# ecml-peagnn/graph_recsys_benchmark

Hardware: AMD Instinct MI355X
Metric: BPR-scored edges/sec, PEAGAT MovieLens-25m, emb_dim=64, 9 metapaths (higher is better)
Workload: dtype f32; 1 GPU; ml25m_shaped PEAGAT forward+BPR: N=273744 nodes, 9 metapaths x 2 steps, 208376439 messages/step, emb 64 / hidden 64 / repr 16, batch 4096 triples; headline=True, parallelism=single

## Files before the change

graph_recsys_benchmark_amd/_lib.py:

```python
import ctypes as C
import os

_HERE = os.path.dirname(os.path.abspath(__file__))
LIB_PATH = os.environ.get('PEA_LIB') or os.path.join(_HERE, 'csrc', 'libpeahip.so')

PEA_OK = 0
KIND_GAT, KIND_GCN, KIND_SAGE = 0, 1, 2
PLAN_SELF_LOOPS = 1
PLAN_EDGE_IDS = 2
FUSE_ATT, FUSE_MEAN = 0, 1
KG_KGAT, KG_KGCN = 0, 1

_ERR_NAMES = {-1: 'bad argument', -2: 'id out of range', -3: 'HIP runtime error', -4: 'workspace too small',
              -5: 'no gfx950 device'}


class PeaError(RuntimeError):
    def __init__(self, code, msg):
        super().__init__('peahip error %d (%s): %s' % (code, _ERR_NAMES.get(code, '?'), msg))
        self.code = code


class ModelDesc(C.Structure):
    _fields_ = [('kind', C.c_int), ('num_channels', C.c_int), ('steps', C.POINTER(C.c_int)),
# ... 9 lines not shown
                ('src_col', C.c_int)]


class GwJob(C.Structure):
    _fields_ = [('a', C.c_void_p), ('lda', C.c_int64), ('ma', C.c_int), ('b', C.c_void_p), ('ldb', C.c_int64),
                ('nb', C.c_int), ('out', C.c_void_p), ('ldo', C.c_int64), ('b_mask', C.c_void_p), ('b_alt', C.c_void_p),
                ('ldb_alt', C.c_int64), ('b_alt_scale', C.c_void_p)]


class XchgJob(C.Structure):
    _fields_ = [('table', C.c_void_p), ('ld', C.c_int64), ('col', C.c_int), ('width', C.c_int), ('nodes', C.c_void_p),
                ('slots', C.c_void_p), ('n', C.c_int64), ('buf_off', C.c_int64), ('slots_per_rank', C.c_int)]


class DenseJob(C.Structure):
    _fields_ = [('a', C.c_void_p), ('lda', C.c_int64), ('k', C.c_int), ('w', C.c_void_p), ('ldw', C.c_int64),
                ('n_out', C.c_int), ('out', C.c_void_p), ('ldo', C.c_int64), ('gate', C.c_void_p), ('ld_gate', C.c_int64)]


class DenseRouteEntry(C.Structure):
    _fields_ = [('name', C.c_char * 32), ('family', C.c_int), ('variant', C.c_int), ('listed', C.c_int), ('col_group', C.c_int),
                ('lds_bytes', C.c_int64), ('n_jobs', C.c_int), ('job', C.c_int * 12), ('col0', C.c_int * 12),
                ('n_out', C.c_int * 12), ('gate_col0', C.c_int * 12)]


class Mlp2BwdChan(C.Structure):
    _fields_ = [('w0', C.c_void_p), ('w1', C.c_void_p), ('dt1_col', C.c_int), ('h_col', C.c_int), ('dz_col', C.c_int),
                ('da_col', C.c_int)]


class Mlp2BwdChanSage(C.Structure):
    _fields_ = [('w0_root', C.c_void_p), ('w1_root', C.c_void_p), ('dr1_col', C.c_int), ('dxr_col', C.c_int)]


class StageOpts(C.Structure):
    _fields_ = [('part', C.c_int), ('sel_ids', C.c_void_p), ('sel_stride', C.c_int64), ('n_sel', C.c_int64),
                ('sel_out', C.c_void_p), ('err_flag', C.c_void_p)]


PART_ALL, PART_SOURCES, PART_REST = 0, 1, 2
BWD_PREMASKED = 0x100

_vp, _i64, _int, _sz = C.c_void_p, C.c_int64, C.c_int, C.c_size_t
SIGNATURES = {
    'pea_version': (C.c_char_p, []),
    'pea_last_error': (C.c_char_p, []),
# ... 40 lines not shown
    'pea_edge_softmax_backward': (_int, [_vp, _int, _vp, _vp, _vp, _vp, _sz, _vp]),
    'pea_kg_edge_types': (_int, [_vp, _int, _vp, _i64, _int, _vp, _vp]),
    'pea_kg_attention_workspace_bytes': (_sz, [_vp, _int, _int, _int]),
    'pea_kg_attention': (_int, [_vp, _int, _int, _int, _vp, _i64, _vp, _vp, _vp, _vp, _vp, _sz, _vp]),
    'pea_grad_weight_workspace_bytes': (_sz, []),
    'pea_grad_weight': (_int, [_i64, _int, C.POINTER(GwJob), _vp, _sz, _vp]),
    'pea_dense_batch': (_int, [_i64, _int, C.POINTER(DenseJob), _vp]),
    'pea_mlp2_backward_data_workspace_bytes': (_sz, [_int, _int, _int, _int]),
    'pea_mlp2_backward_data': (_int, [_i64, _int, C.POINTER(Mlp2BwdChan), _int, _int, _int, _vp, _i64, _vp, _i64, _vp, _i64, _vp,
                                      _i64, _vp, _vp, _int, _vp, _sz, _vp]),
    'pea_rows_nonzero_workspace_bytes': (_sz, [_i64]),
    'pea_rows_nonzero': (_int, [_i64, _int, _vp, _i64, _vp, _vp, _vp, _vp, _sz, _vp]),
    'pea_rows_nonzero_or': (_int, [_i64, _int, _vp, _i64, _vp, _vp, _vp, _vp, _vp, _sz, _vp]),
    'pea_mlp2_backward_data_sage': (_int, [_i64, _int, C.POINTER(Mlp2BwdChan), C.POINTER(Mlp2BwdChanSage), _int, _int, _int,
                                           _vp, _i64, _vp, _i64, _vp, _i64, _vp, _i64, _vp, _i64, _vp, _i64, _vp, _vp, _vp, _sz,
                                           _vp]),
    'pea_grad_weight_rows': (_int, [_i64, _vp, _vp, _i64, _int, C.POINTER(GwJob), _vp, _sz, _vp]),
    'pea_model_set_active_rows0': (_int, [_vp, _vp, _vp, _vp]),
    'pea_rows_zero': (_int, [_vp, _i64, _int, _vp, _vp, _vp]),
    'pea_block_sum': (_int, [_i64, _int, _int, _vp, _i64, _vp, _i64, _vp]),
    'pea_grad_weight_sharded': (_int, [_i64, _int, _int, _int, _int, C.POINTER(GwJob), _vp, _sz, _vp]),
    'pea_dense_batch_rows': (_int, [_i64, _vp, _int, C.POINTER(DenseJob), _vp]),
    'pea_dense_route': (_int, [_i64, _int, _int, C.POINTER(DenseJob), _int, C.POINTER(DenseRouteEntry), C.POINTER(_int)]),
    'pea_sample_negatives': (_int, [_i64, _int, _vp, _vp, _i64, _i64, _vp, _i64, C.c_uint64, C.c_uint32, _vp, _i64, _vp, _vp]),
    'pea_fuse': (_int, [_i64, _int, _int, _vp, _i64, C.POINTER(_int), _vp, _int, _int, _vp, _vp]),
    'pea_bpr_workspace_bytes': (_sz, [_i64]),
    'pea_bpr_score': (_int, [_i64, _int, _i64, _vp, _vp, _i64, _vp, _vp, _vp, _vp, _vp, _vp, _vp, _vp, _sz, _vp]),
    'pea_predict': (_int, [_i64, _int, _i64, _vp, _vp, _vp, _vp, _vp, _vp, _vp, _vp, _vp]),
    'pea_profile_enable': (_int, [_int]),
    'pea_profile_read': (_int, [_int, C.c_char_p, C.POINTER(C.c_float), C.POINTER(C.c_double), C.POINTER(_int)]),
    'pea_profile_read_ex': (_int, [_int, C.c_char_p, C.POINTER(C.c_float), C.POINTER(C.c_double), C.POINTER(C.c_double),
                                   C.POINTER(C.c_double), C.POINTER(_int)]),
    'pea_entity_reg_workspace_bytes': (C.c_size_t, [_i64, _int]),
    'pea_entity_reg': (_int, [_i64, _int, _i64, _vp, _i64, _vp, _i64, _vp, _vp, _vp, C.c_size_t, _vp]),
    'pea_bpr_train_workspace_bytes': (C.c_size_t, [_i64]),
    'pea_bpr_train_supported': (_int, [_int, _int]),
    'pea_bpr_train': (_int, [_i64, _int, _int, _vp, _i64, _vp, _vp, _vp, _vp, _vp, _vp, _vp, _vp, _vp, _vp, _vp, C.c_size_t, _vp]),
    'pea_rows_scatter_sum_workspace_bytes': (C.c_size_t, [_i64]),
    'pea_rows_scatter_sum': (_int, [_i64, _vp, _vp, _i64, _int, _int, C.POINTER(_int), _vp, _i64, _i64, _vp, C.c_size_t, _vp]),
    'pea_rows_pack': (_int, [_vp, _i64, _int, _int, _vp, _i64, _vp, _i64, _vp]),
    'pea_rows_unpack': (_int, [_vp, _i64, _vp, _int, _vp, _i64, _vp, _i64, _int, _vp]),
    'pea_rows_pack_batch': (_int, [_int, C.POINTER(XchgJob), _vp, _vp]),
    'pea_rows_unpack_batch': (_int, [_int, C.POINTER(XchgJob), _vp, _i64, _vp]),
    'pea_rows_select_owned': (_int, [_vp, _i64, _int, _i64, _vp, _i64, _i64, _int, _int, _int, _vp, _vp, _vp]),
    'pea_rank_eval': (_int, [_i64, _int, _int, _i64, _vp, _vp, _vp, _vp, _vp, _vp, _vp, _vp, _vp, _vp, _vp, _vp]),
    'pea_fuse_ablate': (_int, [_i64, _int, _int, _vp, _i64, C.POINTER(_int), _vp, _int, _vp, _vp, _vp]),
# ... 28 lines not shown
            fn.argtypes = args
        _lib = lib
    return _lib


def last_error():
    return load().pea_last_error().decode()


def check(rc):
    if rc != PEA_OK:
        raise PeaError(rc, last_error())


def dense_route(n_rows, rows_given, jobs):
    lib = load()
    cnt = C.c_int()
    check(lib.pea_dense_route(n_rows, int(rows_given), len(jobs), jobs, 0, None, C.byref(cnt)))
    out = (DenseRouteEntry * max(cnt.value, 1))()
    check(lib.pea_dense_route(n_rows, int(rows_given), len(jobs), jobs, cnt.value, out, C.byref(cnt)))
    return list(out[:cnt.value])


def require_device():
    lib = load()
    if lib.pea_device_count() <= 0:
        raise PeaError(-5, 'no gfx950 (MI355X) device visible; the HIP path has no CPU fallback')
    return lib


class Tape:

    def __init__(self):
        self._h = C.c_void_p()
        check(load().pea_tape_create(C.byref(self._h)))

    def record(self):
        return _TapeRecording(self)

    def replay(self):
        check(load().pea_tape_replay(self._h, current_stream()))

    def __len__(self):
        return int(load().pea_tape_length(self._h))

    def __del__(self):
# ... 37 lines not shown
```

graph_recsys_benchmark_amd/csrc/agg.hip:

```cpp
#include <algorithm>
#include <cstdlib>

#include "agg_common.h"

namespace pea {

namespace {

template <int MODE>
__device__ __forceinline__ void finish_row(const AggGroup &P, int row, int c4, int deg, Soft st, float4 sum) {
    float4 o;
    if (MODE == AGG_GAT) {
        const float inv = 1.0f / (st.s + 1e-16f);
        o = scale4(st.acc, inv);
        if (P.stats && c4 % P.F == 0) {
            float *sp = P.stats + (size_t)row * P.ld_stats + 2 * (c4 / P.F);
            sp[0] = st.m;
            sp[1] = st.s;
        }
    } else if (MODE == AGG_GCN || MODE == AGG_WSUM) {
        o = sum;
    } else {
        const float inv = 1.0f / (float)(deg < 1 ? 1 : deg);
        o = scale4(sum, inv);
// ... 237 lines not shown
        }
    }
    if (sub == 0 && active) finish_row<MODE>(P, row, c4, it.end - it.beg, st, sum);
}

template <int G, int MODE, int F4T>
__global__ __launch_bounds__(kBlock) void agg_rows_kernel(const AggLaunch L) {
    if ((int)blockIdx.x >= L.n_long_blocks) {
        const int b = (int)blockIdx.x - L.n_long_blocks;
        int gi = 0;
        while (gi + 1 < L.n_groups && b >= L.blk_short[gi + 1]) ++gi;
        short_rows<G, MODE, F4T>(L.g[gi], b - L.blk_short[gi]);
        return;
    }
    const int gi = find_group(L);
    const AggGroup &P = L.g[gi];
    const int wave = (int)threadIdx.x / kWave;
    const int lane = (int)threadIdx.x % kWave;
    const int item = ((int)blockIdx.x - L.blk_start[gi]) * (kBlock / kWave) + wave;
    if (item >= P.n_long) return;
    const LongItem it = P.long_items[item];
    if (it.slot == -2) return;
    long_item<G, MODE, F4T, 4, false>(P, it, lane, nullptr, nullptr);
}

template <int G, int MODE, int HL, int V4>
__device__ __forceinline__ void long_item_fat(const AggGroup &P, const LongItem it, const int lane) {
    constexpr int NSG = kWave / G, U = 4, V = 4 * V4;
    const int sub = lane / G, sl = lane % G;
    const bool active = sl * V < P.W;
    const int pos = sl % HL;
    const int c0 = active ? (sl / HL) * P.F + 4 * pos : 0;
    constexpr int CS = 4 * HL;
    const float *feat = P.feat + c0;
    const float *feat_self = P.feat_self + c0;
    const int row = it.row;
    const int kk = 2 * (c0 / P.F);

    float sm = kNegBig, ss = 0.f;
    float4 acc[V4];
#pragma unroll
    for (int v = 0; v < V4; ++v) acc[v] = make_float4(0.f, 0.f, 0.f, 0.f);
    float a_d = 0.f, di = 0.f;
    const float slope = P.neg_slope;
    float4 att_s[V4], h_self[V4];
    if (MODE == AGG_GAT) {
// ... 252 lines not shown
        } else if (MODE == AGG_GCN) {
            const float di = P.dinv_self[row];
            sum = fma4(di * di, h, sum);
        }
    }
    const int deg = P.rowptr[row + 1] - P.rowptr[row];
    if (sub == 0 && active) finish_row<MODE>(P, row, c4, deg, st, sum);
}


template <int G, int MODE>
const char *kname(int which) {
    static char names[4][32];
    static bool init = false;
    if (!init) {
        const char *w[4] = {"short", "rows", "merge", "longhot"};
        const char *m = MODE == AGG_GAT ? "gat" : MODE == AGG_GCN ? "gcn" : MODE == AGG_WSUM ? "wsum" : "mean";
        for (int i = 0; i < 4; ++i) snprintf(names[i], sizeof(names[i]), "agg_%s_g%d_%s", w[i], G, m);
        init = true;
    }
    return names[which];
}

template <int G, int MODE, int F4T>
int launch_for_g(const AggLaunch &base, const int *sel, int n_sel, hipStream_t stream) {
    AggLaunch L;
    double bytes_short = 0.0;
    double pull_short = 0.0, table = 0.0;
    for (int i = 0; i < n_sel; ++i) {
        const AggGroup &g = base.g[sel[i]];
        const double per_msg = 4.0 * g.W + 4.0 * g.idx_share + (MODE == AGG_GAT ? 4.0 * (g.W / g.F) : MODE == AGG_GCN ? 4.0 * g.idx_share : 0.0);
        bytes_short += per_msg * g.msgs_short;
        const double pull = 4.0 * g.W + 4.0 + (MODE == AGG_GCN ? 4.0 : 0.0);
        pull_short += pull * g.msgs_short;
        table = table > g.table_rows * 4.0 * g.W ? table : g.table_rows * 4.0 * g.W;
    }
    L.n_groups = 0;
    int blocks = 0, sblocks = 0;
    double pull_plain = 0.0, alg_plain = 0.0;
    for (int i = 0; i < n_sel; ++i) {
        const AggGroup &g = base.g[sel[i]];
        const bool long_here = g.n_long > 0 && !g.hot_col && !g.skip_long;
        if (g.n_short <= 0 && !long_here) continue;
        L.blk_start[L.n_groups] = blocks;
        L.blk_short[L.n_groups] = sblocks;
        AggGroup &c = L.g[L.n_groups++];
        c = g;
        if (!long_here) c.n_long = 0;
        if (g.n_short > 0) sblocks += (g.n_short + (kBlock / G) - 1) / (kBlock / G);
        if (!long_here) continue;
        blocks += ((g.n_long + 3) / 4 + 7) / 8 * 8;
        const double per_msg = 4.0 * g.W + 4.0 * g.idx_share + (MODE == AGG_GAT ? 4.0 * (g.W / g.F) : MODE == AGG_GCN ? 4.0 * g.idx_share : 0.0);
        alg_plain += per_msg * g.msgs_long;
        pull_plain += (4.0 * g.W + 4.0 + (MODE == AGG_GCN ? 4.0 : 0.0)) * g.msgs_long;
    }
    L.blk_start[L.n_groups] = blocks;
    L.blk_short[L.n_groups] = sblocks;
    L.n_long_blocks = blocks;
    if (blocks + sblocks > 0) {
        ProfScope ps(kname<G, MODE>(1), stream, alg_plain + bytes_short, pull_plain + pull_short, table);
        PEA_LAUNCH((agg_rows_kernel<G, MODE, F4T>), dim3(blocks + sblocks), dim3(kBlock), 0, stream, L);
        PEA_HIP(hipGetLastError());
    }
    for (int i = 0; i < n_sel; ++i) {
        const AggGroup &g = base.g[sel[i]];
        if (g.n_long <= 0 || !g.hot_col || g.skip_long) continue;
        if (MODE == AGG_WSUM) return PEA_ERR_ARG;
        L.n_groups = 1;
        L.blk_start[0] = 0;
        L.g[0] = g;
        const size_t lds = (size_t)g.hot_K * g.W * sizeof(float) + (MODE == AGG_GCN ? (size_t)g.hot_K * sizeof(float) : 0);
        static size_t lds_set = 0;
        if (lds > lds_set) {
            PEA_HIP(hipFuncSetAttribute(reinterpret_cast<const void *>(&agg_long_hot_kernel<G, MODE, F4T>),
                                        hipFuncAttributeMaxDynamicSharedMemorySize, (int)lds));
            lds_set = lds;
        }
        const int n_virtual = (g.n_long + 3) / 4;
        const int grid = std::max(8, std::min(256, (n_virtual + 3) / 4 + 7 & ~7));
        const double per_msg = 4.0 * g.W + 4.0 * g.idx_share + (MODE == AGG_GAT ? 4.0 * (g.W / g.F) : MODE == AGG_GCN ? 4.0 * g.idx_share : 0.0);
        const double pull = (4.0 * g.W + (MODE == AGG_GCN ? 4.0 : 0.0)) * g.msgs_long * (1.0 - g.hot_frac) + 4.0 * g.msgs_long +
                            (double)grid * (double)lds;
        ProfScope ps(kname<G, MODE>(3), stream, per_msg * g.msgs_long, pull, g.table_rows * 4.0 * g.W);
        PEA_LAUNCH((agg_long_hot_kernel<G, MODE, F4T>), dim3(grid), dim3(kHotBlock), lds, stream, L);
        PEA_HIP(hipGetLastError());
    }
    L.n_groups = 0;
    blocks = 0;
    for (int i = 0; i < n_sel; ++i) {
        const AggGroup &g = base.g[sel[i]];
        if (g.n_hub <= 0) continue;
        L.blk_start[L.n_groups] = blocks;
        L.g[L.n_groups++] = g;
        blocks += (g.n_hub + 3) / 4;
    }
    L.blk_start[L.n_groups] = blocks;
    if (blocks > 0) {
        ProfScope ps(kname<G, MODE>(2), stream, 0.0);
        PEA_LAUNCH((agg_merge_kernel<G, MODE, F4T>), dim3(blocks), dim3(kBlock), 0, stream, L);
        PEA_HIP(hipGetLastError());
    }
    return PEA_OK;
}

int f4_class(int mode, int G, int F) {
    if (mode != AGG_GAT) return 0;
    const int f4 = F / 4;
    return f4 == G ? G : f4 == 4 ? 4 : 0;
}

template <int G, int MODE>
int launch_g(const AggLaunch &base, int cls, const int *sel, int n, hipStream_t stream) {
    if (MODE == AGG_GAT && cls == G) return launch_for_g<G, MODE, G>(base, sel, n, stream);
    if (MODE == AGG_GAT && cls == 4) return launch_for_g<G, MODE, (G >= 4 ? 4 : 0)>(base, sel, n, stream);
    return launch_for_g<G, MODE, 0>(base, sel, n, stream);
}

template <int MODE>
const char *fat_name(int G) {
    static char names[4][32];
    const int i = G == 8 ? 0 : G == 16 ? 1 : G == 32 ? 2 : 3;
    if (!names[i][0]) {
        const char *m = MODE == AGG_GAT ? "gat" : MODE == AGG_GCN ? "gcn" : "mean";
        snprintf(names[i], sizeof(names[i]), "agg_long_fat_g%d_%s", G, m);
    }
    return names[i];
}

template <int G, int MODE, int HL, int V4>
int launch_fat(const AggLaunch &base, const int *sel, int n_sel, hipStream_t stream) {
    AggLaunch L;
    L.n_groups = 0;
    int blocks = 0;
    double alg = 0.0, pull = 0.0, table = 0.0;
    for (int i = 0; i < n_sel; ++i) {
        const AggGroup &g = base.g[sel[i]];
        L.blk_start[L.n_groups] = blocks;
        L.g[L.n_groups++] = g;
// ... 32 lines not shown
    }
    for (int c = 0; c < 6; ++c) {
        int sel[kMaxAggGroups], n = 0;
        for (int i = 0; i < base.n_groups; ++i)
            if (cls[i] == c) sel[n++] = i;
        if (!n) continue;
        switch (c) {
            case 0: PEA_TRY((launch_fat<8, MODE, 8, 2>(base, sel, n, stream))); break;
            case 1: PEA_TRY((launch_fat<16, MODE, 8, 2>(base, sel, n, stream))); break;
            case 2: PEA_TRY((launch_fat<32, MODE, 8, 2>(base, sel, n, stream))); break;
            case 3: PEA_TRY((launch_fat<8, MODE, 8, 4>(base, sel, n, stream))); break;
            case 4: PEA_TRY((launch_fat<16, MODE, 8, 4>(base, sel, n, stream))); break;
            default: PEA_TRY((launch_fat<16, MODE, 16, 4>(base, sel, n, stream))); break;
        }
        for (int q = 0; q < n; ++q) base.g[sel[q]].skip_long = 1;
    }
    return PEA_OK;
}

template <int MODE>
int launch_mode(const AggLaunch &base_in, hipStream_t stream) {
    AggLaunch base = base_in;
    PEA_TRY(launch_fat_groups<MODE>(base, stream));
    const int classes[3] = {0, 4, -1};
    for (int G = 4; G <= 64; G <<= 1) {
        for (int ci = 0; ci < 3; ++ci) {
            const int cls = classes[ci] < 0 ? G : classes[ci];
            if (ci == 1 && G == 4) continue;
            int sel[kMaxAggGroups], n = 0;
            for (int i = 0; i < base.n_groups; ++i)
                if (lanes_for(base.g[i].W) == G && f4_class(MODE, G, base.g[i].F) == cls) sel[n++] = i;
            if (!n) continue;
            switch (G) {
                case 4: PEA_TRY((launch_g<4, MODE>(base, cls, sel, n, stream))); break;
                case 8: PEA_TRY((launch_g<8, MODE>(base, cls, sel, n, stream))); break;
                case 16: PEA_TRY((launch_g<16, MODE>(base, cls, sel, n, stream))); break;
                case 32: PEA_TRY((launch_g<32, MODE>(base, cls, sel, n, stream))); break;
                default: PEA_TRY((launch_g<64, MODE>(base, cls, sel, n, stream))); break;
            }
        }
    }
    return PEA_OK;
}

}

size_t partial_record_floats(int W, int F) { return (size_t)W + 2 * (size_t)(W / F); }

int launch_aggregate(AggMode mode, const AggGroup *groups, int n_groups, hipStream_t stream) {
    PEA_REQUIRE(n_groups >= 0 && n_groups <= kMaxAggGroups, PEA_ERR_ARG, "aggregate: %d groups (max %d)",
                n_groups, kMaxAggGroups);
    AggLaunch base;
    base.n_groups = n_groups;
    for (int i = 0; i < n_groups; ++i) {
        const AggGroup &g = groups[i];
        PEA_REQUIRE(g.W > 0 && g.W <= 256 && g.W % 4 == 0, PEA_ERR_ARG,
                    "aggregate: group width %d must be a multiple of 4 in (0, 256]", g.W);
        PEA_REQUIRE(g.F > 0 && g.F % 4 == 0 && g.W % g.F == 0, PEA_ERR_ARG,
                    "aggregate: head width %d must be a multiple of 4 dividing %d", g.F, g.W);
        PEA_REQUIRE(g.ld_feat % 4 == 0 && g.ld_out % 4 == 0, PEA_ERR_ARG,
                    "aggregate: row strides must be multiples of 4 floats");
        PEA_REQUIRE(g.n_hub == 0 || g.partial != nullptr, PEA_ERR_ARG, "aggregate: hub rows need a partial buffer");
        PEA_REQUIRE(mode != AGG_GAT || (g.neg_slope >= 0.f && g.neg_slope <= 1.f), PEA_ERR_ARG,
                    "aggregate: negative_slope %g outside [0, 1] is not supported", (double)g.neg_slope);
        base.g[i] = g;
    }
    switch (mode) {
        case AGG_GAT: return launch_mode<AGG_GAT>(base, stream);
        case AGG_GCN: return launch_mode<AGG_GCN>(base, stream);
        case AGG_WSUM: return launch_mode<AGG_WSUM>(base, stream);
        default: return launch_mode<AGG_MEAN>(base, stream);
    }
}

}
```

graph_recsys_benchmark_amd/csrc/agg_common.h:

```cpp
#pragma once
#include "common.h"

namespace pea {
namespace {

constexpr int kBlock = 256;
constexpr float kNegBig = -3.0e38f;
constexpr float kLog2e = 1.44269504088896340736f;

struct AggLaunch {
    int n_groups;
    int blk_start[kMaxAggGroups + 1];
    int n_long_blocks;
    int blk_short[kMaxAggGroups + 1];
    AggGroup g[kMaxAggGroups];
};

__device__ __forceinline__ float4 ld4(const float *p) { return *reinterpret_cast<const float4 *>(p); }
__device__ __forceinline__ void st4(float *p, float4 v) { *reinterpret_cast<float4 *>(p) = v; }
__device__ __forceinline__ float4 fma4(float w, float4 h, float4 a) {
    return make_float4(fmaf(w, h.x, a.x), fmaf(w, h.y, a.y), fmaf(w, h.z, a.z), fmaf(w, h.w, a.w));
}
__device__ __forceinline__ float4 scale4(float4 a, float f) { return make_float4(a.x * f, a.y * f, a.z * f, a.w * f); }
__device__ __forceinline__ float4 add4(float4 a, float4 b) { return make_float4(a.x + b.x, a.y + b.y, a.z + b.z, a.w + b.w); }
__device__ __forceinline__ float4 shfl_xor4(float4 v, int m) {
    return make_float4(__shfl_xor(v.x, m), __shfl_xor(v.y, m), __shfl_xor(v.z, m), __shfl_xor(v.w, m));
}

struct Soft {
    float m, s;
    float4 acc;
    __device__ __forceinline__ void init() { m = kNegBig; s = 0.f; acc = make_float4(0.f, 0.f, 0.f, 0.f); }
    __device__ __forceinline__ void push(float e, float4 h) {
        const float mn = fmaxf(m, e * kLog2e);
        const float fs = __builtin_amdgcn_exp2f(m - mn);
        const float p = __builtin_amdgcn_exp2f(fmaf(e, kLog2e, -mn));
        m = mn;
// ... 66 lines not shown
```

graph_recsys_benchmark_amd/csrc/common.h:

```cpp
#pragma once
#include <hip/hip_runtime.h>

#include <cstdarg>
#include <cstdint>
#include <cstdio>
#include <functional>
#include <string>
#include <vector>

#include "../../include/peahip.h"

namespace pea {

void set_error(const char *fmt, ...);
const char *get_error();

#define PEA_HIP(call)                                                                          \
    do {                                                                                       \
        hipError_t e_ = (call);                                                                \
        if (e_ != hipSuccess) {                                                                \
            pea::set_error("%s:%d: %s failed: %s", __FILE__, __LINE__, #call,                 \
                           hipGetErrorString(e_));                                             \
            return PEA_ERR_HIP;                                                                \
        }                                                                                      \
// ... 187 lines not shown
    m.rank = rank;
    if ((tile & (tile - 1)) == 0) {
        m.shift = 0;
        while ((1 << m.shift) < tile) ++m.shift;
    }
    const int64_t tiles = (N + tile - 1) / tile;
    const int64_t own_tiles = tiles > rank ? (tiles - rank + world - 1) / world : 0;
    m.n = own_tiles * tile;
    return m;
}

inline RowMap make_rowmap_list(int64_t N, const int *list, const int *count_dev, int64_t capacity) {
    RowMap m;
    m.N = N;
    m.n = capacity;
    m.list = list;
    m.count = count_dev;
    return m;
}

constexpr int kMaxAggGroups = 16;
int launch_aggregate(AggMode mode, const AggGroup *groups, int n_groups, hipStream_t stream);
size_t partial_record_floats(int W, int F);
constexpr int kColsumParts = 512;
int launch_gat_backward(AggMode mode, const AggGroup *groups, int n_groups, hipStream_t stream);
int launch_colsum(const RowMap &rows, int W, int F, const float *A, int lda, const float *S, int lds, float scale, float *part,
                  float *out, hipStream_t stream);
int launch_colsum2(const RowMap &rows, int W, int F, const float *A, int lda, const float *S0, const float *S1, int lds,
                   float scale, float *part, float *out0, float *out1, hipStream_t stream);
int launch_relu_mask(const RowMap &rows, int W, float *G, int ldg, const float *O, int ldo, hipStream_t stream);

struct GemmSegment {
    int c0, c1;
    float *dst;
    int ld;
    int relu;
    const float *gate;
    int ld_gate;
};
constexpr int kMaxSegments = 4;
struct GemmJob {
    const unsigned char *a1_mask;
    const float *a1_alt, *a1_bias, *a1_scale;
    int lda_alt;
    const float *A1;
    const float *A2;
// ... 120 lines not shown
```

include/peahip.h:

```cpp
#ifndef PEAHIP_H_
#define PEAHIP_H_

#include <stddef.h>
#include <stdint.h>

#ifdef __cplusplus
extern "C" {
#endif

#define PEA_OK 0
#define PEA_ERR_ARG (-1)
#define PEA_ERR_RANGE (-2)
#define PEA_ERR_HIP (-3)
#define PEA_ERR_NOMEM (-4)
#define PEA_ERR_DEVICE (-5)

#define PEA_KIND_GAT 0
#define PEA_KIND_GCN 1
#define PEA_KIND_SAGE 2

#define PEA_PLAN_SELF_LOOPS 1

#define PEA_PLAN_EDGE_IDS 2

// ... 92 lines not shown
int pea_block_sum(int64_t n_rows, int n_blocks, int width, const float *src, int64_t ld, float *dst, int64_t ld_dst,
                  void *stream);
int pea_grad_weight_sharded(int64_t n_rows, int shard_tile, int shard_world, int shard_rank, int n_jobs,
                            const pea_gw_job *jobs_host, void *workspace, size_t workspace_bytes, void *stream);
int pea_dense_batch_rows(int64_t n_rows, const int32_t *rows, int n_jobs, const pea_dense_job *jobs_host, void *stream);
#define PEA_ROUTE_SKINNY 0
#define PEA_ROUTE_PERSIST 1
#define PEA_ROUTE_DEEP_RESIDENT 2
#define PEA_ROUTE_DEEP_CHUNK 3
#define PEA_ROUTE_DEEP_STAGED 4
#define PEA_ROUTE_MAX_JOBS 12
typedef struct pea_dense_route_entry {
    char name[32];
    int family, variant;
    int listed;
    int col_group;
    int64_t lds_bytes;
    int n_jobs;
    int job[PEA_ROUTE_MAX_JOBS], col0[PEA_ROUTE_MAX_JOBS], n_out[PEA_ROUTE_MAX_JOBS], gate_col0[PEA_ROUTE_MAX_JOBS];
} pea_dense_route_entry;
int pea_dense_route(int64_t n_rows, int rows_given, int n_jobs, const pea_dense_job *jobs_host, int cap,
                    pea_dense_route_entry *entries_out, int *count_out);

int pea_sample_negatives(int64_t n_pos, int k, const int64_t *pos_u, const int64_t *pos_i, int64_t item_lo,
                         int64_t num_items, const int64_t *seen_keys_sorted, int64_t n_keys, uint64_t seed,
                         uint32_t offset, int64_t *out_triples, int64_t ld_out, int *exhausted, void *stream);

typedef struct pea_exchange_desc {
    int relation;
    int64_t slots_per_rank;
    int width;
    int dst_ld;
    size_t dst_offset_bytes;
    size_t src_offset_bytes;
    int src_ld, src_col;
} pea_exchange_desc;
int pea_plan_set_owned_rows(pea_plan *plan, const int32_t *rows, int64_t n, void *stream);
int pea_plan_set_sources(pea_plan *plan, int relation, const int32_t *slot_of_node, int64_t slots_per_rank,
                         const int32_t *need_rows, int64_t n_need, void *stream);
int pea_model_num_stages(const pea_model *model);
int pea_model_forward_stage(pea_model *model, int stage, const float *const *params_host, const float *x,
                            const float *att, int masked_channel, void *workspace, size_t workspace_bytes,
                            float *out_repr, float *out_stack, void *stream);
int pea_model_forward_stage_train(pea_model *model, int stage, const float *const *params_host, const float *x,
                                  const float *att, int masked_channel, void *workspace, size_t workspace_bytes,
                                  float *out_repr, float *out_stack, void *stream);
// ... 154 lines not shown
```

profiles/summarize.py:

```python
#!/usr/bin/env python3
import collections
import csv
import glob
import json
import os
import re
import sys


def short(name):
    m = re.search(r'(agg_\w+_kernel)<(\d+), *(\d+)(?:, *\d+)?>', name)
    if m:
        mode = {'0': 'gat', '1': 'gcn', '2': 'mean'}[m.group(3)]
        return '%s_g%s_%s' % (m.group(1).replace('_kernel', ''), m.group(2), mode)
    m = re.search(r'bwd_(rows|merge)_kernel<(\d+), *(\d+)', name)
    if m:
        side = 'dst' if m.group(3) == '3' else 'src'
        fam = 'sum_bwd' if m.group(3) == '6' else 'gat_bwd'
        return '%s_%s_g%s' % (fam, side, m.group(2)) if m.group(1) == 'rows' else '%s_%s_merge' % (fam, side)
    m = re.search(r'mlp2_kernel<\d+, *\d+, *(true|false|0|1)>', name)
    if m:
        return 'mlp2_kernel_train' if m.group(1) in ('true', '1') else 'mlp2_kernel'
    m = re.search(r'(gemm_mfma|gemm_persist|gemm_skinny)_kernel<(\d+)', name)
    if m:
        return '%s_k%s' % (m.group(1), m.group(2))
    m = re.search(r'pea::\(anonymous namespace\)::(\w+)', name)
    return m.group(1) if m else name[:48]


def main(root):
    out = {}
    f = glob.glob(os.path.join(root, 'stats', '*', '*_kernel_stats.csv'))
    if f:
# ... 76 lines not shown
```

Measured before the change: 129.7 billion edges/s.

## Fuse two lane-width aggregation row launches per level into one pair kernel

Adds a planner that groups aggregation work by lane width and head class. When the two widest classes form a listed pair (GAT or GCN at 32/64 lanes plus 8 lanes), their long-row and short-row blocks run in a single agg_rows_pair_kernel launch, dispatched by block-range tables. This removes one kernel launch and its tail per level, and lets the narrow-class blocks fill the device alongside the wide ones. The trade-off is a per-block group search, a larger launch struct and more template instantiations. The pairing can be turned off with PEA_LEVEL_PAIR=0.

```diff
diff --git a/graph_recsys_benchmark_amd/_lib.py b/graph_recsys_benchmark_amd/_lib.py
--- a/graph_recsys_benchmark_amd/_lib.py
+++ b/graph_recsys_benchmark_amd/_lib.py
@@ -55,6 +55,20 @@
     _fields_ = [('name', C.c_char * 32), ('family', C.c_int), ('variant', C.c_int), ('listed', C.c_int), ('col_group', C.c_int),
                 ('lds_bytes', C.c_int64), ('n_jobs', C.c_int), ('job', C.c_int * 12), ('col0', C.c_int * 12),
                 ('n_out', C.c_int * 12), ('gate_col0', C.c_int * 12)]
+
+
+class LevelGroup(C.Structure):
+    _fields_ = [('width', C.c_int), ('head_width', C.c_int), ('n_short', C.c_int), ('n_long', C.c_int), ('n_hub', C.c_int),
+                ('hot', C.c_int), ('fat', C.c_int)]
+
+
+class LevelLaunch(C.Structure):
+    _fields_ = [('kind', C.c_int), ('lanes', C.c_int * 2), ('head_class', C.c_int * 2), ('n_groups', C.c_int),
+                ('first_b', C.c_int), ('group', C.c_int * 16), ('long_here', C.c_int * 16), ('blk_start', C.c_int * 17),
+                ('blk_short', C.c_int * 17), ('range', C.c_int * 4), ('blocks', C.c_int)]
+
+
+LEVEL_ROWS, LEVEL_PAIR, LEVEL_HOT, LEVEL_MERGE = 0, 1, 2, 3
 
 
 class Mlp2BwdChan(C.Structure):
@@ -141,6 +155,8 @@
     'pea_grad_weight_sharded': (_int, [_i64, _int, _int, _int, _int, C.POINTER(GwJob), _vp, _sz, _vp]),
     'pea_dense_batch_rows': (_int, [_i64, _vp, _int, C.POINTER(DenseJob), _vp]),
     'pea_dense_route': (_int, [_i64, _int, _int, C.POINTER(DenseJob), _int, C.POINTER(DenseRouteEntry), C.POINTER(_int)]),
+    'pea_level_route': (_int, [_int, _int, C.POINTER(LevelGroup), _int, _int, C.POINTER(LevelLaunch), C.POINTER(_int)]),
+    'pea_level_pair_launches': (_i64, []),
     'pea_sample_negatives': (_int, [_i64, _int, _vp, _vp, _i64, _i64, _vp, _i64, C.c_uint64, C.c_uint32, _vp, _i64, _vp, _vp]),
     'pea_fuse': (_int, [_i64, _int, _int, _vp, _i64, C.POINTER(_int), _vp, _int, _int, _vp, _vp]),
     'pea_bpr_workspace_bytes': (_sz, [_i64]),
@@ -215,6 +231,15 @@
     return list(out[:cnt.value])
 
 
+def level_route(mode, groups, allow_pair=True):
+    lib = load()
+    cnt = C.c_int()
+    check(lib.pea_level_route(mode, len(groups), groups, int(allow_pair), 0, None, C.byref(cnt)))
+    out = (LevelLaunch * max(cnt.value, 1))()
+    check(lib.pea_level_route(mode, len(groups), groups, int(allow_pair), cnt.value, out, C.byref(cnt)))
+    return list(out[:cnt.value])
+
+
 def require_device():
     lib = load()
     if lib.pea_device_count() <= 0:
diff --git a/graph_recsys_benchmark_amd/csrc/agg.hip b/graph_recsys_benchmark_amd/csrc/agg.hip
--- a/graph_recsys_benchmark_amd/csrc/agg.hip
+++ b/graph_recsys_benchmark_amd/csrc/agg.hip
@@ -1,5 +1,7 @@
 #include <algorithm>
+#include <atomic>
 #include <cstdlib>
+#include <vector>
 
 #include "agg_common.h"
 
@@ -283,6 +285,37 @@
     const LongItem it = P.long_items[item];
     if (it.slot == -2) return;
     long_item<G, MODE, F4T, 4, false>(P, it, lane, nullptr, nullptr);
+}
+
+template <int MODE, int GA, int FA, int GB, int FB>
+__global__ __launch_bounds__(kBlock) __attribute__((amdgpu_waves_per_eu(8))) void agg_rows_pair_kernel(const AggLaunch L) {
+    const int b = (int)blockIdx.x;
+    if (b >= L.blk_range[2]) {
+        const bool is_b = b >= L.blk_range[3];
+        const int sb = b - L.blk_range[2], hi = is_b ? L.n_groups : L.first_b;
+        int gi = is_b ? L.first_b : 0;
+        while (gi + 1 < hi && sb >= L.blk_short[gi + 1]) ++gi;
+        if (is_b)
+            short_rows<GB, MODE, FB>(L.g[gi], sb - L.blk_short[gi]);
+        else
+            short_rows<GA, MODE, FA>(L.g[gi], sb - L.blk_short[gi]);
+        return;
+    }
+    const bool is_b = b >= L.blk_range[1];
+    const int hi = is_b ? L.n_groups : L.first_b;
+    int gi = is_b ? L.first_b : 0;
+    while (gi + 1 < hi && b >= L.blk_start[gi + 1]) ++gi;
+    const AggGroup &P = L.g[gi];
+    const int wave = (int)threadIdx.x / kWave;
+    const int lane = (int)threadIdx.x % kWave;
+    const int item = (b - L.blk_start[gi]) * (kBlock / kWave) + wave;
+    if (item >= P.n_long) return;
+    const LongItem it = P.long_items[item];
+    if (it.slot == -2) return;
+    if (is_b)
+        long_item<GB, MODE, FB, 4, false>(P, it, lane, nullptr, nullptr);
+    else
+        long_item<GA, MODE, FA, 4, false>(P, it, lane, nullptr, nullptr);
 }
 
 template <int G, int MODE, int HL, int V4>
@@ -581,53 +614,148 @@
     return names[which];
 }
 
+int f4_class(int mode, int G, int F) {
+    if (mode != AGG_GAT) return 0;
+    const int f4 = F / 4;
+    return f4 == G ? G : f4 == 4 ? 4 : 0;
+}
+
+#define PEA_LEVEL_PAIRS(X) X(AGG_GAT, 32, 4, 8, 4) X(AGG_GAT, 64, 4, 8, 4) X(AGG_GCN, 32, 0, 8, 0) X(AGG_GCN, 64, 0, 8, 0)
+
+static_assert(kMaxAggGroups == PEA_LEVEL_MAX_GROUPS, "pea_level_launch holds one entry per group of a level");
+
+struct LevelGroup {
+    int W, F, n_short, n_long, n_hub;
+    bool hot, skip_long;
+};
+
+bool pair_listed(int mode, int ga, int fa, int gb, int fb) {
+#define PEA_PAIR_TEST(m, a, x, b, y) \
+    if (mode == m && ga == a && fa == x && gb == b && fb == y) return true;
+    PEA_LEVEL_PAIRS(PEA_PAIR_TEST)
+#undef PEA_PAIR_TEST
+    return false;
+}
+
+void add_class_rows(pea_level_launch &E, const LevelGroup *g, const int *sel, int n, int G) {
+    int blocks = E.blk_start[E.n_groups], sblocks = E.blk_short[E.n_groups];
+    for (int i = 0; i < n; ++i) {
+        const LevelGroup &q = g[sel[i]];
+        const bool long_here = q.n_long > 0 && !q.hot && !q.skip_long;
+        if (q.n_short <= 0 && !long_here) continue;
+        E.group[E.n_groups] = sel[i];
+        E.long_here[E.n_groups] = long_here;
+        if (q.n_short > 0) sblocks += (q.n_short + (kBlock / G) - 1) / (kBlock / G);
+        if (long_here) blocks += ((q.n_long + 3) / 4 + 7) / 8 * 8;
+        ++E.n_groups;
+        E.blk_start[E.n_groups] = blocks;
+        E.blk_short[E.n_groups] = sblocks;
+    }
+}
+
+void plan_level_launches(int mode, const LevelGroup *g, int n_groups, bool allow_pair, std::vector<pea_level_launch> *plan) {
+    struct Class {
+        int G, cls, n, sel[kMaxAggGroups];
+    };
+    std::vector<Class> classes;
+    const int order[3] = {0, 4, -1};
+    for (int G = 4; G <= 64; G <<= 1) {
+        for (int ci = 0; ci < 3; ++ci) {
+            if (ci == 1 && G == 4) continue;
+            Class c;
+            c.G = G, c.cls = order[ci] < 0 ? G : order[ci], c.n = 0;
+            for (int i = 0; i < n_groups; ++i)
+                if (lanes_for(g[i].W) == G && f4_class(mode, G, g[i].F) == c.cls) c.sel[c.n++] = i;
+            if (c.n) classes.push_back(c);
+        }
+    }
+    int pa = -1, pb = -1;
+    bool plain = true;
+    for (int i = 0; i < n_groups; ++i) plain = plain && !g[i].hot && !g[i].skip_long;
+    if (allow_pair && plain && classes.size() >= 2) {
+        const Class &A = classes[classes.size() - 1], &B = classes[classes.size() - 2];
+        if (pair_listed(mode, A.G, A.cls, B.G, B.cls)) {
+            pea_level_launch E{};
+            E.kind = PEA_LEVEL_PAIR;
+            E.lanes[0] = A.G, E.head_class[0] = A.cls, E.lanes[1] = B.G, E.head_class[1] = B.cls;
+            add_class_rows(E, g, A.sel, A.n, A.G);
+            E.first_b = E.n_groups;
+            add_class_rows(E, g, B.sel, B.n, B.G);
+            if (E.first_b > 0 && E.n_groups > E.first_b) {
+                E.range[0] = 0;
+                E.range[1] = E.blk_start[E.first_b];
+                E.range[2] = E.blk_start[E.n_groups];
+                E.range[3] = E.range[2] + E.blk_short[E.first_b];
+                E.blocks = E.range[2] + E.blk_short[E.n_groups];
+                plan->push_back(E);
+                pa = (int)classes.size() - 1, pb = (int)classes.size() - 2;
+            }
+        }
+    }
+    for (int k = 0; k < (int)classes.size(); ++k) {
+        const Class &c = classes[k];
+        pea_level_launch E{};
+        E.lanes[0] = c.G, E.head_class[0] = c.cls;
+        if (k != pa && k != pb) {
+            E.kind = PEA_LEVEL_ROWS;
+            add_class_rows(E, g, c.sel, c.n, c.G);
+            E.first_b = E.n_groups;
+            E.range[1] = E.range[2] = E.blk_start[E.n_groups];
+            E.range[3] = E.blocks = E.range[2] + E.blk_short[E.n_groups];
+            if (E.blocks > 0) plan->push_back(E);
+        }
+        for (int i = 0; i < c.n; ++i) {
+            const LevelGroup &q = g[c.sel[i]];
+            if (q.n_long <= 0 || !q.hot || q.skip_long) continue;
+            E = pea_level_launch{};
+            E.kind = PEA_LEVEL_HOT;
+            E.lanes[0] = c.G, E.head_class[0] = c.cls;
+            E.n_groups = E.first_b = 1;
+            E.group[0] = c.sel[i];
+            E.long_here[0] = 1;
+            const int n_virtual = (q.n_long + 3) / 4;
+            E.blocks = std::max(8, std::min(256, ((n_virtual + 3) / 4 + 7) & ~7));
+            plan->push_back(E);
+        }
+        E = pea_level_launch{};
+        E.kind = PEA_LEVEL_MERGE;
+        E.lanes[0] = c.G, E.head_class[0] = c.cls;
+        for (int i = 0; i < c.n; ++i) {
+            const LevelGroup &q = g[c.sel[i]];
+            if (q.n_hub <= 0) continue;
+            E.group[E.n_groups++] = c.sel[i];
+            E.blk_start[E.n_groups] = E.blk_start[E.n_groups - 1] + (q.n_hub + 3) / 4;
+        }
+        E.first_b = E.n_groups;
+        E.blocks = E.blk_start[E.n_groups];
+        if (E.blocks > 0) plan->push_back(E);
+    }
+}
+
+std::atomic<long> g_pair_launches{0};
+
+template <int MODE>
+double alg_per_msg(const AggGroup &g) {
+    return 4.0 * g.W + 4.0 * g.idx_share + (MODE == AGG_GAT ? 4.0 * (g.W / g.F) : MODE == AGG_GCN ? 4.0 * g.idx_share : 0.0);
+}
+
 template <int G, int MODE, int F4T>
-int launch_for_g(const AggLaunch &base, const int *sel, int n_sel, hipStream_t stream) {
-    AggLaunch L;
-    double bytes_short = 0.0;
-    double pull_short = 0.0, table = 0.0;
-    for (int i = 0; i < n_sel; ++i) {
-        const AggGroup &g = base.g[sel[i]];
-        const double per_msg = 4.0 * g.W + 4.0 * g.idx_share + (MODE == AGG_GAT ? 4.0 * (g.W / g.F) : MODE == AGG_GCN ? 4.0 * g.idx_share : 0.0);
-        bytes_short += per_msg * g.msgs_short;
-        const double pull = 4.0 * g.W + 4.0 + (MODE == AGG_GCN ? 4.0 : 0.0);
-        pull_short += pull * g.msgs_short;
-        table = table > g.table_rows * 4.0 * g.W ? table : g.table_rows * 4.0 * g.W;
-    }
-    L.n_groups = 0;
-    int blocks = 0, sblocks = 0;
-    double pull_plain = 0.0, alg_plain = 0.0;
-    for (int i = 0; i < n_sel; ++i) {
-        const AggGroup &g = base.g[sel[i]];
-        const bool long_here = g.n_long > 0 && !g.hot_col && !g.skip_long;
-        if (g.n_short <= 0 && !long_here) continue;
-        L.blk_start[L.n_groups] = blocks;
-        L.blk_short[L.n_groups] = sblocks;
-        AggGroup &c = L.g[L.n_groups++];
-        c = g;
-        if (!long_here) c.n_long = 0;
-        if (g.n_short > 0) sblocks += (g.n_short + (kBlock / G) - 1) / (kBlock / G);
-        if (!long_here) continue;
-        blocks += ((g.n_long + 3) / 4 + 7) / 8 * 8;
-        const double per_msg = 4.0 * g.W + 4.0 * g.idx_share + (MODE == AGG_GAT ? 4.0 * (g.W / g.F) : MODE == AGG_GCN ? 4.0 * g.idx_share : 0.0);
-        alg_plain += per_msg * g.msgs_long;
-        pull_plain += (4.0 * g.W + 4.0 + (MODE == AGG_GCN ? 4.0 : 0.0)) * g.msgs_long;
-    }
-    L.blk_start[L.n_groups] = blocks;
-    L.blk_short[L.n_groups] = sblocks;
-    L.n_long_blocks = blocks;
-    if (blocks + sblocks > 0) {
-        ProfScope ps(kname<G, MODE>(1), stream, alg_plain + bytes_short, pull_plain + pull_short, table);
-        PEA_LAUNCH((agg_rows_kernel<G, MODE, F4T>), dim3(blocks + sblocks), dim3(kBlock), 0, stream, L);
+int issue_level_launch(const pea_level_launch &E, AggLaunch &L, hipStream_t stream) {
+    if (E.kind == PEA_LEVEL_ROWS) {
+        double alg = 0.0, pull = 0.0, table = 0.0;
+        for (int q = 0; q < L.n_groups; ++q) {
+            const AggGroup &g = L.g[q];
+            const double msgs = g.msgs_short + (E.long_here[q] ? g.msgs_long : 0.0);
+            alg += alg_per_msg<MODE>(g) * msgs;
+            pull += (4.0 * g.W + 4.0 + (MODE == AGG_GCN ? 4.0 : 0.0)) * msgs;
+            table = std::max(table, g.table_rows * 4.0 * g.W);
+        }
+        ProfScope ps(kname<G, MODE>(1), stream, alg, pull, table);
+        PEA_LAUNCH((agg_rows_kernel<G, MODE, F4T>), dim3(E.blocks), dim3(kBlock), 0, stream, L);
         PEA_HIP(hipGetLastError());
-    }
-    for (int i = 0; i < n_sel; ++i) {
-        const AggGroup &g = base.g[sel[i]];
-        if (g.n_long <= 0 || !g.hot_col || g.skip_long) continue;
+    } else if (E.kind == PEA_LEVEL_HOT) {
         if (MODE == AGG_WSUM) return PEA_ERR_ARG;
-        L.n_groups = 1;
-        L.blk_start[0] = 0;
-        L.g[0] = g;
+        const AggGroup &g = L.g[0];
         const size_t lds = (size_t)g.hot_K * g.W * sizeof(float) + (MODE == AGG_GCN ? (size_t)g.hot_K * sizeof(float) : 0);
         static size_t lds_set = 0;
         if (lds > lds_set) {
@@ -635,44 +763,51 @@
                                         hipFuncAttributeMaxDynamicSharedMemorySize, (int)lds));
             lds_set = lds;
         }
-        const int n_virtual = (g.n_long + 3) / 4;
-        const int grid = std::max(8, std::min(256, (n_virtual + 3) / 4 + 7 & ~7));
-        const double per_msg = 4.0 * g.W + 4.0 * g.idx_share + (MODE == AGG_GAT ? 4.0 * (g.W / g.F) : MODE == AGG_GCN ? 4.0 * g.idx_share : 0.0);
         const double pull = (4.0 * g.W + (MODE == AGG_GCN ? 4.0 : 0.0)) * g.msgs_long * (1.0 - g.hot_frac) + 4.0 * g.msgs_long +
-                            (double)grid * (double)lds;
-        ProfScope ps(kname<G, MODE>(3), stream, per_msg * g.msgs_long, pull, g.table_rows * 4.0 * g.W);
-        PEA_LAUNCH((agg_long_hot_kernel<G, MODE, F4T>), dim3(grid), dim3(kHotBlock), lds, stream, L);
+                            (double)E.blocks * (double)lds;
+        ProfScope ps(kname<G, MODE>(3), stream, alg_per_msg<MODE>(g) * g.msgs_long, pull, g.table_rows * 4.0 * g.W);
+        PEA_LAUNCH((agg_long_hot_kernel<G, MODE, F4T>), dim3(E.blocks), dim3(kHotBlock), lds, stream, L);
         PEA_HIP(hipGetLastError());
-    }
-    L.n_groups = 0;
-    blocks = 0;
-    for (int i = 0; i < n_sel; ++i) {
-        const AggGroup &g = base.g[sel[i]];
-        if (g.n_hub <= 0) continue;
-        L.blk_start[L.n_groups] = blocks;
-        L.g[L.n_groups++] = g;
-        blocks += (g.n_hub + 3) / 4;
-    }
-    L.blk_start[L.n_groups] = blocks;
-    if (blocks > 0) {
+    } else {
         ProfScope ps(kname<G, MODE>(2), stream, 0.0);
-        PEA_LAUNCH((agg_merge_kernel<G, MODE, F4T>), dim3(blocks), dim3(kBlock), 0, stream, L);
+        PEA_LAUNCH((agg_merge_kernel<G, MODE, F4T>), dim3(E.blocks), dim3(kBlock), 0, stream, L);
         PEA_HIP(hipGetLastError());
     }
     return PEA_OK;
 }
 
-int f4_class(int mode, int G, int F) {
-    if (mode != AGG_GAT) return 0;
-    const int f4 = F / 4;
-    return f4 == G ? G : f4 == 4 ? 4 : 0;
-}
-
 template <int G, int MODE>
-int launch_g(const AggLaunch &base, int cls, const int *sel, int n, hipStream_t stream) {
-    if (MODE == AGG_GAT && cls == G) return launch_for_g<G, MODE, G>(base, sel, n, stream);
-    if (MODE == AGG_GAT && cls == 4) return launch_for_g<G, MODE, (G >= 4 ? 4 : 0)>(base, sel, n, stream);
-    return launch_for_g<G, MODE, 0>(base, sel, n, stream);
+int issue_g(const pea_level_launch &E, AggLaunch &L, hipStream_t stream) {
+    const int cls = E.head_class[0];
+    if (MODE == AGG_GAT && cls == G) return issue_level_launch<G, MODE, G>(E, L, stream);
+    if (MODE == AGG_GAT && cls == 4) return issue_level_launch<G, MODE, (G >= 4 ? 4 : 0)>(E, L, stream);
+    return issue_level_launch<G, MODE, 0>(E, L, stream);
+}
+
+template <int MODE>
+int issue_pair(const pea_level_launch &E, AggLaunch &L, hipStream_t stream) {
+    double alg = 0.0, pull = 0.0, table = 0.0;
+    for (int q = 0; q < L.n_groups; ++q) {
+        const AggGroup &g = L.g[q];
+        const double msgs = g.msgs_short + (E.long_here[q] ? g.msgs_long : 0.0);
+        alg += alg_per_msg<MODE>(g) * msgs;
+        pull += (4.0 * g.W + 4.0 + (MODE == AGG_GCN ? 4.0 : 0.0)) * msgs;
+        table = std::max(table, g.table_rows * 4.0 * g.W);
+    }
+#define PEA_PAIR_ISSUE(m, a, x, b, y)                                                                                   \
+    if constexpr (MODE == m) {                                                                                          \
+        if (E.lanes[0] == a && E.head_class[0] == x && E.lanes[1] == b && E.head_class[1] == y) {                       \
+            ProfScope ps(kname<a, MODE>(1), stream, alg, pull, table);                                                  \
+            PEA_LAUNCH((agg_rows_pair_kernel<MODE, a, x, b, y>), dim3(E.blocks), dim3(kBlock), 0, stream, L);           \
+            PEA_HIP(hipGetLastError());                                                                                 \
+            g_pair_launches.fetch_add(1, std::memory_order_relaxed);                                                    \
+            return PEA_OK;                                                                                              \
+        }                                                                                                               \
+    }
+    PEA_LEVEL_PAIRS(PEA_PAIR_ISSUE)
+#undef PEA_PAIR_ISSUE
+    PEA_REQUIRE(false, PEA_ERR_ARG, "aggregate: no pair kernel for lanes %d + %d", E.lanes[0], E.lanes[1]);
+    return PEA_OK;
 }
 
 template <int MODE>
@@ -751,22 +886,35 @@
 int launch_mode(const AggLaunch &base_in, hipStream_t stream) {
     AggLaunch base = base_in;
     PEA_TRY(launch_fat_groups<MODE>(base, stream));
-    const int classes[3] = {0, 4, -1};
-    for (int G = 4; G <= 64; G <<= 1) {
-        for (int ci = 0; ci < 3; ++ci) {
-            const int cls = classes[ci] < 0 ? G : classes[ci];
-            if (ci == 1 && G == 4) continue;
-            int sel[kMaxAggGroups], n = 0;
-            for (int i = 0; i < base.n_groups; ++i)
-                if (lanes_for(base.g[i].W) == G && f4_class(MODE, G, base.g[i].F) == cls) sel[n++] = i;
-            if (!n) continue;
-            switch (G) {
-                case 4: PEA_TRY((launch_g<4, MODE>(base, cls, sel, n, stream))); break;
-                case 8: PEA_TRY((launch_g<8, MODE>(base, cls, sel, n, stream))); break;
-                case 16: PEA_TRY((launch_g<16, MODE>(base, cls, sel, n, stream))); break;
-                case 32: PEA_TRY((launch_g<32, MODE>(base, cls, sel, n, stream))); break;
-                default: PEA_TRY((launch_g<64, MODE>(base, cls, sel, n, stream))); break;
-            }
+    LevelGroup lg[kMaxAggGroups];
+    for (int i = 0; i < base.n_groups; ++i) {
+        const AggGroup &g = base.g[i];
+        lg[i] = LevelGroup{g.W, g.F, g.n_short, g.n_long, g.n_hub, g.hot_col != nullptr, g.skip_long != 0};
+    }
+    const char *env = getenv("PEA_LEVEL_PAIR");
+    std::vector<pea_level_launch> plan;
+    plan_level_launches(MODE, lg, base.n_groups, !(env && atoi(env) == 0), &plan);
+    for (const pea_level_launch &E : plan) {
+        AggLaunch L;
+        L.n_groups = E.n_groups;
+        L.first_b = E.first_b;
+        L.n_long_blocks = E.range[2];
+        for (int q = 0; q < 4; ++q) L.blk_range[q] = E.range[q];
+        for (int q = 0; q <= E.n_groups; ++q) L.blk_start[q] = E.blk_start[q], L.blk_short[q] = E.blk_short[q];
+        for (int q = 0; q < E.n_groups; ++q) {
+            L.g[q] = base.g[E.group[q]];
+            if (E.kind != PEA_LEVEL_MERGE && !E.long_here[q]) L.g[q].n_long = 0;
+        }
+        if (E.kind == PEA_LEVEL_PAIR) {
+            PEA_TRY(issue_pair<MODE>(E, L, stream));
+            continue;
+        }
+        switch (E.lanes[0]) {
+            case 4: PEA_TRY((issue_g<4, MODE>(E, L, stream))); break;
+            case 8: PEA_TRY((issue_g<8, MODE>(E, L, stream))); break;
+            case 16: PEA_TRY((issue_g<16, MODE>(E, L, stream))); break;
+            case 32: PEA_TRY((issue_g<32, MODE>(E, L, stream))); break;
+            default: PEA_TRY((issue_g<64, MODE>(E, L, stream))); break;
         }
     }
     return PEA_OK;
@@ -775,6 +923,30 @@
 }
 
 size_t partial_record_floats(int W, int F) { return (size_t)W + 2 * (size_t)(W / F); }
+
+int level_route(int mode, int n_groups, const pea_level_group *groups, bool allow_pair, int cap, pea_level_launch *entries,
+                int *count) {
+    PEA_REQUIRE(mode == AGG_GAT || mode == AGG_GCN || mode == AGG_MEAN || mode == AGG_WSUM, PEA_ERR_ARG,
+                "level_route: mode %d is not a forward aggregation", mode);
+    PEA_REQUIRE(n_groups >= 0 && n_groups <= kMaxAggGroups, PEA_ERR_ARG, "level_route: %d groups (max %d)", n_groups,
+                kMaxAggGroups);
+    LevelGroup lg[kMaxAggGroups];
+    for (int i = 0; i < n_groups; ++i) {
+        const pea_level_group &g = groups[i];
+        PEA_REQUIRE(g.width > 0 && g.width <= 256 && g.width % 4 == 0 && g.head_width > 0 && g.head_width % 4 == 0 &&
+                        g.width % g.head_width == 0,
+                    PEA_ERR_ARG, "level_route: group %d has width %d, head width %d", i, g.width, g.head_width);
+        PEA_REQUIRE(g.n_short >= 0 && g.n_long >= 0 && g.n_hub >= 0, PEA_ERR_ARG, "level_route: group %d has a negative count", i);
+        lg[i] = LevelGroup{g.width, g.head_width, g.n_short, g.n_long, g.n_hub, g.hot != 0, g.fat != 0};
+    }
+    std::vector<pea_level_launch> plan;
+    plan_level_launches(mode, lg, n_groups, allow_pair, &plan);
+    *count = (int)plan.size();
+    for (int i = 0; i < (int)plan.size() && i < cap; ++i) entries[i] = plan[i];
+    return PEA_OK;
+}
+
+long level_pair_launches() { return g_pair_launches.load(std::memory_order_relaxed); }
 
 int launch_aggregate(AggMode mode, const AggGroup *groups, int n_groups, hipStream_t stream) {
     PEA_REQUIRE(n_groups >= 0 && n_groups <= kMaxAggGroups, PEA_ERR_ARG, "aggregate: %d groups (max %d)",
@@ -803,3 +975,12 @@
 }
 
 }
+
+extern "C" int pea_level_route(int mode, int n_groups, const pea_level_group *groups_host, int allow_pair, int cap,
+                               pea_level_launch *entries_out, int *count_out) {
+    PEA_REQUIRE(count_out && cap >= 0 && (entries_out || cap == 0) && (groups_host || n_groups == 0), PEA_ERR_ARG,
+                "level_route: bad arguments");
+    return pea::level_route(mode, n_groups, groups_host, allow_pair != 0, cap, entries_out, count_out);
+}
+
+extern "C" int64_t pea_level_pair_launches(void) { return (int64_t)pea::level_pair_launches(); }
diff --git a/graph_recsys_benchmark_amd/csrc/agg_common.h b/graph_recsys_benchmark_amd/csrc/agg_common.h
--- a/graph_recsys_benchmark_amd/csrc/agg_common.h
+++ b/graph_recsys_benchmark_amd/csrc/agg_common.h
@@ -13,6 +13,8 @@
     int blk_start[kMaxAggGroups + 1];
     int n_long_blocks;
     int blk_short[kMaxAggGroups + 1];
+    int first_b;
+    int blk_range[4];
     AggGroup g[kMaxAggGroups];
 };
 
diff --git a/graph_recsys_benchmark_amd/csrc/common.h b/graph_recsys_benchmark_amd/csrc/common.h
--- a/graph_recsys_benchmark_amd/csrc/common.h
+++ b/graph_recsys_benchmark_amd/csrc/common.h
@@ -233,6 +233,9 @@
 constexpr int kMaxAggGroups = 16;
 int launch_aggregate(AggMode mode, const AggGroup *groups, int n_groups, hipStream_t stream);
 size_t partial_record_floats(int W, int F);
+int level_route(int mode, int n_groups, const pea_level_group *groups, bool allow_pair, int cap, pea_level_launch *entries,
+                int *count);
+long level_pair_launches();
 constexpr int kColsumParts = 512;
 int launch_gat_backward(AggMode mode, const AggGroup *groups, int n_groups, hipStream_t stream);
 int launch_colsum(const RowMap &rows, int W, int F, const float *A, int lda, const float *S, int lds, float scale, float *part,
diff --git a/include/peahip.h b/include/peahip.h
--- a/include/peahip.h
+++ b/include/peahip.h
@@ -138,6 +138,30 @@
 int pea_dense_route(int64_t n_rows, int rows_given, int n_jobs, const pea_dense_job *jobs_host, int cap,
                     pea_dense_route_entry *entries_out, int *count_out);
 
+#define PEA_LEVEL_ROWS 0
+#define PEA_LEVEL_PAIR 1
+#define PEA_LEVEL_HOT 2
+#define PEA_LEVEL_MERGE 3
+#define PEA_LEVEL_MAX_GROUPS 16
+typedef struct pea_level_group {
+    int width, head_width;
+    int n_short, n_long, n_hub;
+    int hot, fat;
+} pea_level_group;
+typedef struct pea_level_launch {
+    int kind;
+    int lanes[2], head_class[2];
+    int n_groups, first_b;
+    int group[PEA_LEVEL_MAX_GROUPS];
+    int long_here[PEA_LEVEL_MAX_GROUPS];
+    int blk_start[PEA_LEVEL_MAX_GROUPS + 1], blk_short[PEA_LEVEL_MAX_GROUPS + 1];
+    int range[4];
+    int blocks;
+} pea_level_launch;
+int pea_level_route(int mode, int n_groups, const pea_level_group *groups_host, int allow_pair, int cap,
+                    pea_level_launch *entries_out, int *count_out);
+int64_t pea_level_pair_launches(void);
+
 int pea_sample_negatives(int64_t n_pos, int k, const int64_t *pos_u, const int64_t *pos_i, int64_t item_lo,
                          int64_t num_items, const int64_t *seen_keys_sorted, int64_t n_keys, uint64_t seed,
                          uint32_t offset, int64_t *out_triples, int64_t ld_out, int *exhausted, void *stream);
diff --git a/profiles/summarize.py b/profiles/summarize.py
--- a/profiles/summarize.py
+++ b/profiles/summarize.py
@@ -9,6 +9,9 @@
 
 
 def short(name):
+    m = re.search(r'agg_rows_pair_kernel<(\d+), *(\d+)', name)
+    if m:
+        return 'agg_rows_g%s_%s' % (m.group(2), {'0': 'gat', '1': 'gcn', '2': 'mean'}[m.group(1)])
     m = re.search(r'(agg_\w+_kernel)<(\d+), *(\d+)(?:, *\d+)?>', name)
     if m:
         mode = {'0': 'gat', '1': 'gcn', '2': 'mean'}[m.group(3)]
```

Result: no change. 129.6 billion edges/s (-0.1%).
